# pyannote/pyannote-audio

Measured on AMD Instinct MI355X. Metric: audio-hours/sec (real-time factor) for speaker-diarization-3.1 pipeline, higher is better.
Workload: dtype f32

## Files before the change

### include/pyannote_amd.h

```cpp
#ifndef PYANNOTE_AMD_H
#define PYANNOTE_AMD_H

#include <stddef.h>
#include <stdint.h>

#ifdef __cplusplus
extern "C" {
#endif

int pa_version(void);
const char* pa_last_error(void);

void pa_prof_enable(int on);
size_t pa_prof_report(char* buf, size_t cap);

#define PA_MAX_LSTM_LAYERS 8
#define PA_MAX_LINEAR 4

typedef struct pa_seg_weights {
  int32_t sinc_stride;
  int32_t lstm_layers;
  int32_t lstm_hidden;
  int32_t lstm_bidir;
  int32_t num_linear;
// ... 66 lines not shown
  int32_t bottleneck;
  const float* fb_window;
  const float* fb_tw256;
  const float* fb_tw512;
  const float* fb_mel_w;
  const int32_t* fb_mel_lo;
  const int32_t* fb_mel_hi;
  const float* stem_w;
  const float* stem_shift;
  const float* blk_w1[PA_MAX_RES_BLOCKS];
  const float* blk_shift1[PA_MAX_RES_BLOCKS];
  const float* blk_w2[PA_MAX_RES_BLOCKS];
  const float* blk_shift2[PA_MAX_RES_BLOCKS];
  const float* blk_u1[PA_MAX_RES_BLOCKS];
  const float* blk_u2[PA_MAX_RES_BLOCKS];
  const float* blk_wsc[PA_MAX_RES_BLOCKS];
  const float* blk_shiftsc[PA_MAX_RES_BLOCKS];
  const float* blk_w3[PA_MAX_RES_BLOCKS];
  const float* blk_shift3[PA_MAX_RES_BLOCKS];
  const float* seg1_w;
  const float* seg1_b;
  const float* blk_v1[PA_MAX_RES_BLOCKS];
  const float* blk_v2[PA_MAX_RES_BLOCKS];
  int32_t fb_center_kernel;
} pa_emb_weights;

int pa_emb_num_fbank_frames(int num_samples);
int pa_emb_num_pool_frames(const pa_emb_weights* w, int num_samples);
size_t pa_emb_workspace_bytes(const pa_emb_weights* w, int num_chunks, int num_samples, int num_masks);
int pa_emb_forward(const pa_emb_weights* w, const float* wav, int64_t wav_len, int64_t chunk_stride,
                   int num_chunks, int num_samples, const float* masks, int num_masks, int mask_frames,
                   const int32_t* nearest_idx, float* emb, void* workspace, size_t workspace_bytes,
                   void* stream);

size_t pa_emb_ragged_workspace_bytes(const pa_emb_weights* w, int num_utterances, int max_samples);
int pa_emb_forward_ragged(const pa_emb_weights* w, const float* wav, int64_t wav_len, const int64_t* offsets,
                          const int32_t* lengths, int num_utterances, int max_samples, const float* masks, float* emb,
                          void* workspace, size_t workspace_bytes, void* stream);

size_t pa_emb_calibrate_workspace_bytes(const pa_emb_weights* w, int num_chunks, int num_samples);
int pa_emb_calibrate_winograd(const pa_emb_weights* w, const float* wav, int64_t wav_len, int64_t chunk_stride,
                              int num_chunks, int num_samples, float* report, float* emb, void* workspace,
                              size_t workspace_bytes, void* stream);
int pa_absmax_diff(const float* got, const float* ref, long n, float* out2, void* stream);

int pa_fbank(const float* wav, long wav_len, long chunk_stride, int B, int N, const float* window,
             const float* tw256, const float* tw512, const float* mel_w, const int* mel_lo,
             const int* mel_hi, int nmel, float* out, int center, void* stream);
int pa_fbank_center_span(const float* fb, int B, int T, int nmel, int kernel, float* out, void* stream);
int pa_resnet_stem(const float* fbank, int B, int T, int F, const float* w9, const float* shift,
                   float* out, void* stream);
int pa_conv3x3(const float* X, int B, int H, int W, int cin, const float* Wg, const float* shift,
               const float* R, float* Y, int cout, int stride, int relu, void* stream);
int pa_winograd_pack_host(const float* conv_weight ,
                          const float* bn_scale , int cout, int cin,
                          float* U_slabs );
int pa_conv3x3_wino(const float* X, int B, int H, int W, int cin, const float* U, const float* shift,
                    const float* R, float* Y, int cout, int relu, void* stream);
int pa_winograd4_pack_host(const float* conv_weight ,
                           const float* bn_scale , int cout, int cin,
                           float* U_slabs );
int pa_conv3x3_wino4(const float* X, int B, int H, int W, int cin, const float* U, const float* shift,
                     const float* R, float* Y, int cout, int relu, void* stream);
int pa_conv3x3_wino4_rows(const float* X, int B, int H, int W, int cin, const float* U, const float* shift,
                          const float* R, float* Y, int cout, int relu, int rows, void* stream);
int pa_conv3x3_wino_rows(const float* X, int B, int H, int W, int cin, const float* U, const float* shift,
                         const float* R, float* Y, int cout, int relu, int y_first, void* stream);
int pa_stats_pool(const float* feat, int B, int Fh, int Tp, int C, const float* masks, int S, int Fm,
                  const int* nearest_idx, float* stats, void* stream);
int pa_fbank_ragged(const float* wav, long wav_len, const int64_t* offsets, const int32_t* lengths, int B,
                    int max_samples, const float* window, const float* tw256, const float* tw512, const float* mel_w,
                    const int* mel_lo, const int* mel_hi, int nmel, float* out, void* stream);
int pa_zero_tail_cols(float* x, int B, int H, int W, int C, const int32_t* lengths, int halvings, void* stream);
int pa_stats_pool_ragged(const float* feat, int B, int Fh, int W, int C, const int32_t* lengths, int halvings,
                         const float* masks, int ld_masks, float* stats, void* stream);

#define PA_W2V_MAX_CONV 8
#define PA_W2V_MAX_LAYERS 24
typedef struct pa_w2v_layer {
  const float* qk_w;
  const float* qk_b;
  const float* v_w;
  const float* out_w;
  const float* out_b;
  const float* ln1_g;
  const float* ln1_b;
  const float* ff1_w;
  const float* ff1_b;
  const float* ff2_w;
  const float* ff2_b;
  const float* ln2_g;
  const float* ln2_b;
  const float* gate_w;
  const float* gate_b;
  const float* gate_const;
} pa_w2v_layer;

typedef struct pa_sser_weights {
  int32_t num_conv;
  int32_t conv_channels[PA_W2V_MAX_CONV];
  int32_t conv_kernel[PA_W2V_MAX_CONV];
  int32_t conv_stride[PA_W2V_MAX_CONV];
  int32_t extractor_layer_norm;
  int32_t embed_dim, num_layers, num_heads, ff_dim, layer_norm_first;
  int32_t pos_kernel, pos_groups;
  int32_t wavlm;
// ... 122 lines not shown
```

### pyannote-audio_amd/csrc/emb_forward.cpp

```cpp
#include <hip/hip_runtime.h>
#include <stdint.h>
#include <stdlib.h>

#include "../../include/pyannote_amd.h"

namespace pa {
void set_error(const char* fmt, ...);
}

namespace {

struct EmbPlan {
  int B, N, T, F, S;
  int Hs[5], Ws[5];
  size_t fbank, act[4], stats, total, act_elems;
  size_t t2_off, gather_off;
};
inline size_t align64(size_t n) { return (n + 63) & ~(size_t)63; }

inline bool prefer_wino4(int H, int W, int cin) {
  auto up = [](int a, int b) { return (long)((a + b - 1) / b) * b; };
  long p4 = up(H, 4) * up(W, 64);
  const long p4_lin = up(H, 4) * up(W, 4);
  if (p4_lin * 120 <= p4 * 100) p4 = p4_lin * 120 / 100;
  long p2 = up(H, 8) * up(W, 32);
  if (up(H, 4) * up(W, 64) < p2) p2 = up(H, 4) * up(W, 64);
  if (up(H, 2) * up(W, 128) < p2) p2 = up(H, 2) * up(W, 128);
  const long gain = cin >= 256 ? 130 : 122;
  return p4 * 100 <= p2 * gain;
}

inline bool split_rows_wanted() {
  static const bool on = getenv("PA_EMB_SPLIT_ROWS") != nullptr && atoi(getenv("PA_EMB_SPLIT_ROWS")) != 0;
  return on;
}

bool make_plan(const pa_emb_weights* w, int B, int N, int S, EmbPlan* p, bool calib = false) {
  if (N < 400) return false;
  p->B = B;
  p->N = N;
  p->S = S < 1 ? 1 : S;
  p->T = 1 + (N - 400) / 160;
  p->F = w->num_mel;
  p->Hs[0] = p->F;
  p->Ws[0] = p->T;
  for (int l = 0; l < w->num_layers; ++l) {
    const int s = l == 0 ? 1 : 2;
    p->Hs[l + 1] = (p->Hs[l] - 1) / s + 1;
    p->Ws[l + 1] = (p->Ws[l] - 1) / s + 1;
  }
  size_t o = 0;
  auto take = [&](size_t n) {
    size_t r = o;
    o += align64(n);
    return r;
  };
  p->fbank = take((size_t)B * p->T * p->F);
  const int ex = w->bottleneck ? 4 : 1;
  p->act_elems = (size_t)B * p->Hs[0] * p->Ws[0] * w->planes[0] * ex;
  for (int i = 0; i < 3; ++i) p->act[i] = take(p->act_elems);
  p->t2_off = p->gather_off = 0;
  if (w->bottleneck) {
    size_t t1 = 0, t2 = 0, g = 0;
    int cin = w->planes[0];
    for (int l = 0; l < w->num_layers; ++l) {
      const size_t planes = w->planes[l];
      const size_t in_px = (size_t)B * p->Hs[l == 0 ? 1 : l] * p->Ws[l == 0 ? 1 : l];
      const size_t out_px = (size_t)B * p->Hs[l + 1] * p->Ws[l + 1];
      t1 = t1 > in_px * planes ? t1 : in_px * planes;
      t2 = t2 > out_px * planes ? t2 : out_px * planes;
      if (l > 0) g = g > out_px * cin ? g : out_px * cin;
      cin = 4 * (int)planes;
    }
    p->t2_off = align64(t1);
    p->gather_off = p->t2_off + align64(t2);
    p->act[3] = take(p->gather_off + align64(g));
  } else if (calib) {
    p->act[3] = take(p->act_elems);
  }
  const int L = w->num_layers;
  p->stats = take((size_t)B * p->S * 2 * w->planes[L - 1] * ex * p->Hs[L]);
  p->total = o;
  return true;
}

}
// ... 108 lines not shown
    for (int l = 0; l < w->num_layers; ++l) {
      const int planes = w->planes[l], cout = 4 * planes;
      for (int i = 0; i < w->num_blocks[l]; ++i, ++blk) {
        if (blk >= PA_MAX_RES_BLOCKS) {
          pa::set_error("pa_emb_forward: more than %d residual blocks", PA_MAX_RES_BLOCKS);
          return 3;
        }
        const int stride = (i == 0 && l > 0) ? 2 : 1;
        const int H = stride == 2 ? p.Hs[l] : p.Hs[l + 1], W = stride == 2 ? p.Ws[l] : p.Ws[l + 1];
        const int Ho = p.Hs[l + 1], Wo = p.Ws[l + 1];
        float* t1 = tmp;
        float* t2 = tmp + p.t2_off;
        RUN(pa_gemm_tn_ex(cur, cin, w->blk_w1[blk], cin, w->blk_shift1[blk], nullptr, t1, planes, B * H * W,
                          planes, cin, 2, 0, stream));
        RUN(zero_tail(t1, stride == 2 ? l : l + 1, planes));
        if (stride == 1 && w->blk_u2[blk] != nullptr)
          RUN(pa_conv3x3_wino(t1, B, H, W, planes, w->blk_u2[blk], w->blk_shift2[blk], nullptr, t2, planes, 1,
                              stream));
        else
          RUN(pa_conv3x3(t1, B, H, W, planes, w->blk_w2[blk], w->blk_shift2[blk], nullptr, t2, planes, stride,
                         1, stream));
        const float* res = cur;
        if (w->blk_wsc[blk] != nullptr) {
          if (stride == 2)
            RUN(pa_gemm_tn_s2(cur, B, H, W, cin, w->blk_wsc[blk], cin, w->blk_shiftsc[blk], sc, cout, cout, stream));
          else
            RUN(pa_gemm_tn_ex(cur, cin, w->blk_wsc[blk], cin, w->blk_shiftsc[blk], nullptr, sc, cout,
                              B * Ho * Wo, cout, cin, 0, 0, stream));
          res = sc;
        } else if (stride != 1 || cin != cout) {
          pa::set_error("pa_emb_forward: block %d needs a shortcut conv but none was given", blk);
          return 3;
        }
        RUN(pa_gemm_tn_ex(t2, planes, w->blk_w3[blk], planes, w->blk_shift3[blk], res, nxt, cout, B * Ho * Wo,
                          cout, planes, 2, 0, stream));
        float* t = cur;
        cur = nxt;
        nxt = t;
        cin = cout;
      }
    }
  } else
  for (int l = 0; l < w->num_layers; ++l) {
    const int cout = w->planes[l];
    for (int i = 0; i < w->num_blocks[l]; ++i, ++blk) {
      if (blk >= PA_MAX_RES_BLOCKS) {
        pa::set_error("pa_emb_forward: more than %d residual blocks", PA_MAX_RES_BLOCKS);
        return 3;
      }
      const int stride = (i == 0 && l > 0) ? 2 : 1;
      const int H = stride == 2 ? p.Hs[l] : p.Hs[l + 1], W = stride == 2 ? p.Ws[l] : p.Ws[l + 1];
      const int Ho = p.Hs[l + 1], Wo = p.Ws[l + 1];
      if (w->blk_wsc[blk] != nullptr) {
        RUN(pa_conv3x3(cur, B, H, W, cin, w->blk_w1[blk], w->blk_shift1[blk], nullptr, f1, cout, stride,
                       1, stream));
        RUN(zero_tail(f1, l + 1, cout));
        const size_t q = (size_t)B * Ho * Wo * cin;
        float* R = f2 + ((q + 63) & ~(size_t)63);
        if (stride == 2)
          RUN(pa_gemm_tn_s2(cur, B, H, W, cin, w->blk_wsc[blk], cin, w->blk_shiftsc[blk], R, cout, cout, stream));
        else
          RUN(pa_gemm_tn(cur, cin, w->blk_wsc[blk], cin, w->blk_shiftsc[blk], R, cout, B * Ho * Wo, cout, cin, 0, 0,
                         stream));
        RUN(conv_s1(f1, Ho, Wo, cout, w->blk_v2[blk], w->blk_u2[blk], w->blk_w2[blk], w->blk_shift2[blk], R, cur, cout,
                    2 * blk + 1));
        RUN(zero_tail(cur, l + 1, cout));
      } else {
        if (stride != 1 || cin != cout) {
          pa::set_error("pa_emb_forward: block %d needs a shortcut conv but none was given", blk);
          return 3;
        }
        RUN(conv_s1(cur, H, W, cin, w->blk_v1[blk], w->blk_u1[blk], w->blk_w1[blk], w->blk_shift1[blk], nullptr, f1,
                    cout, 2 * blk));
        RUN(zero_tail(f1, l + 1, cout));
        RUN(conv_s1(f1, H, W, cout, w->blk_v2[blk], w->blk_u2[blk], w->blk_w2[blk], w->blk_shift2[blk], cur, f2, cout,
                    2 * blk + 1));
        RUN(zero_tail(f2, l + 1, cout));
        float* t = cur;
        cur = f2;
        f2 = t;
      }
      cin = cout;
    }
  }
  const int L = w->num_layers;
  const int S = p.S;
  const int cfin = w->planes[L - 1] * (w->bottleneck ? 4 : 1);
  if (ragged)
    RUN(pa_stats_pool_ragged(cur, B, p.Hs[L], p.Ws[L], cfin, lengths, L - 1, masks, p.Ws[L], ws + p.stats, stream));
  else
    RUN(pa_stats_pool(cur, B, p.Hs[L], p.Ws[L], cfin, masks, S, mask_frames, nearest_idx, ws + p.stats, stream));
  const int D2 = 2 * cfin * p.Hs[L];
  RUN(pa_gemm_tn(ws + p.stats, D2, w->seg1_w, D2, w->seg1_b, emb, w->embed_dim, B * S, w->embed_dim, D2,
                 0, 0, stream));
#undef RUN
  return 0;
}

extern "C" {

int pa_emb_forward(const pa_emb_weights* w, const float* wav, int64_t wav_len, int64_t chunk_stride,
                   int num_chunks, int num_samples, const float* masks, int num_masks, int mask_frames,
                   const int32_t* nearest_idx, float* emb, void* workspace, size_t workspace_bytes,
                   void* stream) {
  return emb_forward_impl(w, wav, wav_len, chunk_stride, num_chunks, num_samples, masks, num_masks, mask_frames,
                          nearest_idx, emb, workspace, workspace_bytes, stream, nullptr);
}

size_t pa_emb_ragged_workspace_bytes(const pa_emb_weights* w, int num_utterances, int max_samples) {
  EmbPlan p;
  if (!make_plan(w, num_utterances, max_samples, 1, &p)) return 0;
  return p.total * sizeof(float);
}

int pa_emb_forward_ragged(const pa_emb_weights* w, const float* wav, int64_t wav_len, const int64_t* offsets,
                          const int32_t* lengths, int num_utterances, int max_samples, const float* masks, float* emb,
// ... 29 lines not shown
```

### pyannote-audio_amd/csrc/emb_resnet.hip

```cpp
#include "common.h"
#ifndef PA_CONV_STORE_AUX
#define PA_CONV_STORE_AUX 0
#endif

namespace pa {

constexpr int STEM_TS = 64;
constexpr int STEM_LD = STEM_TS + 3;

__global__ __launch_bounds__(256) void k_stem(const float* __restrict__ fb, int T, int F,
                                              const float* __restrict__ w9,
                                              const float* __restrict__ shift,
                                              float* __restrict__ out) {
  extern __shared__ float xs[];
  const int b = blockIdx.y, t0 = blockIdx.x * STEM_TS;
  const int tid = threadIdx.x;
  for (int i = tid; i < 2 * STEM_LD; i += 256) xs[(i < STEM_LD ? 0 : (F + 1) * STEM_LD - STEM_LD) + i] = 0.f;
  const int n = (STEM_TS + 2) * F;
  for (int i0 = 0; i0 < n; i0 += 8 * 256) {
    float v[8];
#pragma unroll
    for (int k = 0; k < 8; ++k) {
      const int i = i0 + tid + 256 * k;
      const int tt = i / F, ff = i - tt * F, t = t0 + tt - 1;
// ... 27 lines not shown
  float* o = out + ((long)b * F * T + t0 + pl) * 32 + q4;
  for (int f = 0; f < F; ++f) {
#pragma unroll
    for (int h = 0; h < 2; ++h)
#pragma unroll
      for (int dt = 0; dt < 3; ++dt) x2[h][dt] = xs[(f + 2) * STEM_LD + pl + 32 * h + dt];
    float* of = o + (long)f * T * 32;
#pragma unroll
    for (int h = 0; h < 2; ++h) {
      float acc[4];
#pragma unroll
      for (int c = 0; c < 4; ++c) acc[c] = 0.f;
#pragma unroll
      for (int dt = 0; dt < 3; ++dt)
#pragma unroll
        for (int c = 0; c < 4; ++c) acc[c] = fmaf(x0[h][dt], w[dt][c], acc[c]);
#pragma unroll
      for (int dt = 0; dt < 3; ++dt)
#pragma unroll
        for (int c = 0; c < 4; ++c) acc[c] = fmaf(x1[h][dt], w[3 + dt][c], acc[c]);
#pragma unroll
      for (int dt = 0; dt < 3; ++dt)
#pragma unroll
        for (int c = 0; c < 4; ++c) acc[c] = fmaf(x2[h][dt], w[6 + dt][c], acc[c]);
      float4 o4;
      o4.x = fmaxf(acc[0] + sh[0], 0.f);
      o4.y = fmaxf(acc[1] + sh[1], 0.f);
      o4.z = fmaxf(acc[2] + sh[2], 0.f);
      o4.w = fmaxf(acc[3] + sh[3], 0.f);
      if (h == 0 ? ok0 : ok1) *reinterpret_cast<float4*>(of + 32 * 32 * h) = o4;
    }
#pragma unroll
    for (int h = 0; h < 2; ++h)
#pragma unroll
      for (int dt = 0; dt < 3; ++dt) {
        x0[h][dt] = x1[h][dt];
        x1[h][dt] = x2[h][dt];
      }
  }
}

constexpr int CB = 16;
constexpr int CLD = CB + 4;

template <int S, int TH, int TWT>
struct ConvGeom {
  static constexpr int TW = 32 * TWT;
  static constexpr int PH = (TH - 1) * S + 3;
  static constexpr int PW = (TW - 1) * S + 3;
  static constexpr int PWH = ((TW + 1 + 3) / 8) * 8 + 4;
  static constexpr int PATCH = S == 1 ? PH * PW * CLD : PH * 2 * PWH * CLD;
};

template <int S, int TH, int TWT, int BN, bool HAS_R>
__global__ __launch_bounds__(256, 2) void k_conv3x3(const float* __restrict__ X, int H, int W, int CIN,
                                                    const float* __restrict__ Wg,
                                                    const float* __restrict__ shift,
                                                    const float* __restrict__ R, float* __restrict__ Y,
                                                    int Ho, int Wo, int COUT, int relu, int tiles_w,
                                                    int tiles_hw, int n_tiles, int total_tiles, int xranges,
                                                    int* __restrict__ counters) {
  using G = ConvGeom<S, TH, TWT>;
  constexpr int MT = TH * TWT;
  constexpr int MPW = MT / 4;
  constexpr int NT = BN / 32;
  static_assert(MT % 4 == 0, "M-tiles must split over 4 waves");
  extern __shared__ __attribute__((aligned(16))) float smem[];
  float* patch = smem;
  float* wts = smem + G::PATCH;

  const int tid = threadIdx.x, lane = tid & 63, wv = tid >> 6;
  const int li = lane & 31, kh = lane >> 5;
  constexpr int NPF4 = G::PH * G::PW * (CB / 4);
  constexpr int NP = (NPF4 + 255) / 256;
  constexpr int NWF4 = 9 * BN * (CB / 4);
  constexpr int NW = (NWF4 + 255) / 256;
  constexpr int OOB = (int)0x80000000;

  struct Tile {
    int b, n0, y0, x0;
  };
  const int num_pb = total_tiles / n_tiles;
  auto pair_of = [&](int t) {
    return xranges ? (t & 7) * ((num_pb + 7) >> 3) + (t >> 3) / n_tiles : ((t >> 3) / n_tiles) * 8 + (t & 7);
  };
  auto decode = [&](int t) {
    Tile q;
    const int pb = pair_of(t);
    q.n0 = (((t >> 3) % n_tiles)) * BN;
    const int pix = pb % tiles_hw;
    q.b = pb / tiles_hw;
    q.y0 = (pix / tiles_w) * TH;
    q.x0 = (pix % tiles_w) * G::TW;
    return q;
  };
  auto resolve = [&](const TileQueue& tqq, int r) {
    for (;;) {
      const int t = tq_resolve(tqq, r);
      if (t < 0 || pair_of(t) < num_pb) return t;
      r = tq_claim_own(tqq);
    }
  };
  u32x4 rp[NP], rw[NW];
  constexpr bool HOIST = S == 2;
  struct Offs {
    int p[NP];
  };
  int offw[NW];
#pragma unroll
  for (int e = 0; e < NW; ++e) {
    const int i = tid + 256 * e;
    const int c4 = i & 3, rn = i >> 2;
    const int tap = rn / BN, n = rn % BN;
    offw[e] = (NWF4 % 256 == 0 || i < NWF4) ? ((tap * COUT + n) * CIN + 4 * c4) * 4 : OOB;
  }
  auto tile_offsets = [&](const Tile& q, Offs& o) {
#pragma unroll
    for (int e = 0; e < NP; ++e) {
      const int i = tid + 256 * e;
      const int c4 = i & 3, pp = i >> 2;
      const int py = pp / G::PW, px = pp % G::PW;
      const int iy = q.y0 * S - 1 + py, ix = q.x0 * S - 1 + px;
      o.p[e] = ((NPF4 % 256 == 0 || i < NPF4) && iy >= 0 && iy < H && ix >= 0 && ix < W)
                   ? ((iy * W + ix) * CIN + 4 * c4) * 4
                   : OOB;
    }
  };
  auto gload = [&](const Tile& q, const Offs& o, int c0) {
    const __amdgpu_buffer_rsrc_t xsrd = __builtin_amdgcn_make_buffer_rsrc(
        const_cast<float*>(X + (long)q.b * H * W * CIN), 0, H * W * CIN * 4, 0x00020000);
    const __amdgpu_buffer_rsrc_t wsrd = __builtin_amdgcn_make_buffer_rsrc(
        const_cast<float*>(Wg + (long)q.n0 * CIN), 0, (9 * COUT - q.n0) * CIN * 4, 0x00020000);
    Offs here;
    if (!HOIST) tile_offsets(q, here);
#pragma unroll
    for (int e = 0; e < NP; ++e)
      rp[e] = __builtin_amdgcn_raw_buffer_load_b128(xsrd, HOIST ? o.p[e] : here.p[e], c0 * 4, 0);
#pragma unroll
    for (int e = 0; e < NW; ++e) rw[e] = __builtin_amdgcn_raw_buffer_load_b128(wsrd, offw[e], c0 * 4, 0);
  };
  auto lstore = [&]() {
#pragma unroll
    for (int e = 0; e < NP; ++e) {
      const int i = tid + 256 * e;
      const int c4 = i & 3, pp = i >> 2;
      const int py = pp / G::PW, px = pp % G::PW;
      int off;
      if (S == 1) off = pp * CLD + 4 * c4;
      else off = ((py * 2 + (px & 1)) * G::PWH + (px >> 1)) * CLD + 4 * c4;
      if (NPF4 % 256 == 0 || i < NPF4) *reinterpret_cast<u32x4*>(patch + off) = rp[e];
    }
#pragma unroll
    for (int e = 0; e < NW; ++e) {
      const int i = tid + 256 * e;
      if (NWF4 % 256 == 0 || i < NWF4)
        *reinterpret_cast<u32x4*>(wts + (i >> 2) * CLD + 4 * (i & 3)) = rw[e];
    }
  };

  __shared__ int s_next;
  const TileQueue tq{counters, (int)(blockIdx.x & 7), ((num_pb + 7) >> 3) * n_tiles};
  if (tid == 0) s_next = resolve(tq, tq_claim_own(tq));
  __syncthreads();
  int t = s_next;
  if (t < 0) {
    if (tid == 0) tq_done(tq, gridDim.x);
    return;
  }
  Tile cur = decode(t);
  Offs oc, on;
  if (HOIST) tile_offsets(cur, oc);
  on = oc;
  gload(cur, oc, 0);
  for (;;) {
    int ahead = 0;
    if (tid == 0) ahead = tq_claim_own(tq);
    int tn = -1;
    f32x16 acc[MPW][NT];
#pragma unroll
    for (int i = 0; i < MPW; ++i)
#pragma unroll
      for (int j = 0; j < NT; ++j)
#pragma unroll
        for (int r = 0; r < 16; ++r) acc[i][j][r] = 0.f;
    Tile nxt = cur;

    for (int c0 = 0; c0 < CIN; c0 += CB) {
      __syncthreads();
      lstore();
      if (c0 == 0 && tid == 0) s_next = resolve(tq, ahead);
      __syncthreads();
      if (c0 == 0) {
        tn = s_next;
        if (tn >= 0) {
          nxt = decode(tn);
          if (HOIST) tile_offsets(nxt, on);
        }
      }
      if (c0 + CB < CIN) gload(cur, oc, c0 + CB);
      else if (tn >= 0) gload(nxt, on, 0);
      float4 af[1][MPW][2], bf[1][NT][2];
      auto load_tap = [&](int tap, float4 (&a)[MPW][2], float4 (&bq)[NT][2]) {
        const int dy = tap / 3, dx = tap % 3;
#pragma unroll
        for (int i = 0; i < MPW; ++i) {
          const int mt = wv * MPW + i;
          const int yy = mt / TWT, xt = mt % TWT;
          int off;
          if (S == 1) off = ((yy + dy) * G::PW + 32 * xt + li + dx) * CLD;
          else off = (((yy * 2 + dy) * 2 + (dx & 1)) * G::PWH + 32 * xt + li + (dx >> 1)) * CLD;
          a[i][0] = *reinterpret_cast<const float4*>(patch + off + kh * 8);
          a[i][1] = *reinterpret_cast<const float4*>(patch + off + kh * 8 + 4);
        }
#pragma unroll
        for (int j = 0; j < NT; ++j) {
          const int off = (tap * BN + 32 * j + li) * CLD + kh * 8;
          bq[j][0] = *reinterpret_cast<const float4*>(wts + off);
          bq[j][1] = *reinterpret_cast<const float4*>(wts + off + 4);
        }
      };
      auto mfma_tap = [&](const float4 (&a)[MPW][2], const float4 (&bq)[NT][2]) {
#pragma unroll
        for (int h = 0; h < 2; ++h)
#pragma unroll
          for (int i = 0; i < MPW; ++i)
#pragma unroll
            for (int j = 0; j < NT; ++j) {
              acc[i][j] = MFMA32(a[i][h].x, bq[j][h].x, acc[i][j]);
              acc[i][j] = MFMA32(a[i][h].y, bq[j][h].y, acc[i][j]);
              acc[i][j] = MFMA32(a[i][h].z, bq[j][h].z, acc[i][j]);
              acc[i][j] = MFMA32(a[i][h].w, bq[j][h].w, acc[i][j]);
            }
      };
#pragma unroll 1
      for (int dy = 0; dy < 3; ++dy)
#pragma unroll
        for (int dx = 0; dx < 3; ++dx) {
          load_tap(dy * 3 + dx, af[0], bf[0]);
          mfma_tap(af[0], bf[0]);
        }
    }
    {
      const __amdgpu_buffer_rsrc_t ysrd = __builtin_amdgcn_make_buffer_rsrc(
          Y + (long)cur.b * Ho * Wo * COUT, 0, Ho * Wo * COUT * 4, 0x00020000);
      const __amdgpu_buffer_rsrc_t rsrd = __builtin_amdgcn_make_buffer_rsrc(
          const_cast<float*>(HAS_R ? R + (long)cur.b * Ho * Wo * COUT : Y), 0,
          Ho * Wo * COUT * 4, 0x00020000);
      constexpr int NG = MPW * NT;
      int off[2][16];
      float rv[2][16];
      auto goffs = [&](int g, int* o) {
        const int i = g / NT, j = g % NT;
        const int mt = wv * MPW + i;
        const int y = cur.y0 + mt / TWT, xbase = cur.x0 + 32 * (mt % TWT) + 4 * kh;
        const int n = cur.n0 + 32 * j + li;
#pragma unroll
        for (int r = 0; r < 16; ++r) {
          const int x = xbase + (r & 3) + 8 * (r >> 2);
          o[r] = (y < Ho && x < Wo) ? ((y * Wo + x) * COUT + n) * 4 : OOB;
        }
      };
      auto gres = [&](const int* o, float* v) {
        if (HAS_R) {
#pragma unroll
          for (int r = 0; r < 16; ++r)
            v[r] = __builtin_bit_cast(float, __builtin_amdgcn_raw_buffer_load_b32(rsrd, o[r], 0, 0));
        } else {
#pragma unroll
          for (int r = 0; r < 16; ++r) v[r] = 0.f;
        }
      };
      goffs(0, off[0]);
      gres(off[0], rv[0]);
#pragma unroll
      for (int g = 0; g < NG; ++g) {
        if (g + 1 < NG) {
          goffs(g + 1, off[(g + 1) & 1]);
          gres(off[(g + 1) & 1], rv[(g + 1) & 1]);
        }
        const int i = g / NT, j = g % NT;
        const float sh = shift[cur.n0 + 32 * j + li];
#pragma unroll
        for (int r = 0; r < 16; ++r) {
          float v = acc[i][j][r] + sh + rv[g & 1][r];
          if (relu) v = fmaxf(v, 0.f);
          __builtin_amdgcn_raw_buffer_store_b32(__builtin_bit_cast(unsigned int, v), ysrd,
                                                off[g & 1][r], 0, PA_CONV_STORE_AUX);
        }
      }
    }
    if (tn < 0) break;
    cur = nxt;
    oc = on;
  }
  if (tid == 0) tq_done(tq, gridDim.x);
}

int xcd_ranges_wanted(bool by_default);

template <int S, int TH, int TWT, int BN, bool HAS_R>
static int launch_conv_r(const float* X, int B, int H, int W, int CIN, const float* Wg,
                         const float* shift, const float* R, float* Y, int COUT, int relu,
                         hipStream_t st) {
  using G = ConvGeom<S, TH, TWT>;
  const int Ho = (H - 1) / S + 1, Wo = (W - 1) / S + 1;
  const int tiles_w = cdiv(Wo, G::TW), tiles_h = cdiv(Ho, TH);
  const size_t lds = (size_t)(G::PATCH + 9 * BN * CLD) * sizeof(float);
  constexpr int MAXDEV = 16;
  static int resident_of[MAXDEV] = {0}, per_cu_of[MAXDEV] = {0};
  int dev = 0;
  (void)hipGetDevice(&dev);
  if (dev < 0 || dev >= MAXDEV) dev = 0;
  if (!resident_of[dev]) {
    (void)hipFuncSetAttribute((const void*)k_conv3x3<S, TH, TWT, BN, HAS_R>,
                              hipFuncAttributeMaxDynamicSharedMemorySize, (int)lds);
    int cus = 256, per_cu = 2;
    (void)hipDeviceGetAttribute(&cus, hipDeviceAttributeMultiprocessorCount, dev);
    if (hipOccupancyMaxActiveBlocksPerMultiprocessor(&per_cu, k_conv3x3<S, TH, TWT, BN, HAS_R>, 256, lds) !=
            hipSuccess || per_cu < 1)
      per_cu = 2;
    resident_of[dev] = cus * per_cu;
    per_cu_of[dev] = per_cu;
  }
  const int resident = resident_of[dev] & ~7;
  const int tiles_hw = tiles_w * tiles_h, n_tiles = COUT / BN;
  const long total = (long)tiles_hw * n_tiles * B;
  const int grid = (int)(total < resident ? total : resident);
  int* counters = tile_counters();
  if (counters == nullptr) {
    set_error("pa_conv3x3: cannot allocate the tile counters");
    return 2;
  }
  hipLaunchKernelGGL((k_conv3x3<S, TH, TWT, BN, HAS_R>), dim3(grid), dim3(256), lds, st, X, H, W, CIN, Wg,
                     shift, R, Y, Ho, Wo, COUT, relu, tiles_w, tiles_hw, n_tiles, (int)total, xcd_ranges_wanted(true),
                     counters);
  return 0;
}

template <int S, int TH, int TWT, int BN>
static int launch_conv(const float* X, int B, int H, int W, int CIN, const float* Wg,
                       const float* shift, const float* R, float* Y, int COUT, int relu,
                       hipStream_t st) {
  return R != nullptr ? launch_conv_r<S, TH, TWT, BN, true>(X, B, H, W, CIN, Wg, shift, R, Y, COUT, relu, st)
                      : launch_conv_r<S, TH, TWT, BN, false>(X, B, H, W, CIN, Wg, shift, R, Y, COUT, relu, st);
}

}

extern "C" {

int pa_resnet_stem(const float* fbank, int B, int T, int F, const float* w9, const float* shift,
                   float* out, void* stream) {
  if (B <= 0) return 0;
  pa::ProfScope prof("k_stem", stream, 2.0 * B * T * F * 9 * 32, 4.0 * B * T * F * 33);
  PA_REQUIRE(F >= 1 && (size_t)(F + 2) * pa::STEM_LD * 4 <= 64 * 1024, "pa_resnet_stem: %d mel bins do not fit LDS", F);
  hipLaunchKernelGGL(pa::k_stem, dim3(pa::cdiv(T, pa::STEM_TS), B), dim3(256), (size_t)(F + 2) * pa::STEM_LD * 4,
                     (hipStream_t)stream, fbank, T, F, w9, shift, out);
  PA_CHECK_LAUNCH("pa_resnet_stem");
  return 0;
}

int pa_conv3x3(const float* X, int B, int H, int W, int cin, const float* Wg, const float* shift,
               const float* R, float* Y, int cout, int stride, int relu, void* stream) {
  if (B <= 0) return 0;
  PA_REQUIRE(cin % pa::CB == 0 && cout % 32 == 0, "pa_conv3x3: cin %% 16 and cout %% 32 required");
  hipStream_t st = (hipStream_t)stream;
  const int Ho = (H - 1) / stride + 1, Wo_ = (W - 1) / stride + 1;
  pa::ProfScope prof("k_conv3x3", stream, 2.0 * 9 * cin * cout * (double)B * Ho * Wo_,
                     4.0 * ((double)B * H * W * cin + (double)B * Ho * Wo_ * cout * (R ? 2 : 1) + 9.0 * cin * cout));
  if (stride == 1) {
    if (cout == 32) pa::launch_conv<1, 8, 1, 32>(X, B, H, W, cin, Wg, shift, R, Y, cout, relu, st);
    else if (Ho >= 32) pa::launch_conv<1, 8, 1, 64>(X, B, H, W, cin, Wg, shift, R, Y, cout, relu, st);
    else if (Ho >= 16) pa::launch_conv<1, 4, 2, 64>(X, B, H, W, cin, Wg, shift, R, Y, cout, relu, st);
    else pa::launch_conv<1, 2, 2, 64>(X, B, H, W, cin, Wg, shift, R, Y, cout, relu, st);
  } else if (stride == 2) {
    PA_REQUIRE(cout % 64 == 0, "pa_conv3x3: stride 2 needs cout %% 64 == 0");
    if (Ho >= 16) pa::launch_conv<2, 4, 1, 32>(X, B, H, W, cin, Wg, shift, R, Y, cout, relu, st);
    else pa::launch_conv<2, 2, 2, 32>(X, B, H, W, cin, Wg, shift, R, Y, cout, relu, st);
  } else {
    PA_REQUIRE(false, "pa_conv3x3: stride %d not supported", stride);
  }
  PA_CHECK_LAUNCH("pa_conv3x3");
  return 0;
}

}
```

### pyannote-audio_amd/ffi.py

```python
from __future__ import annotations

import ctypes as C
from pathlib import Path

import torch

_LIB = None
PA_MAX_LSTM_LAYERS = 8
PA_MAX_LINEAR = 4

c_fp = C.c_void_p


class SegWeights(C.Structure):
    _fields_ = [
        ("sinc_stride", C.c_int32), ("lstm_layers", C.c_int32), ("lstm_hidden", C.c_int32),
        ("lstm_bidir", C.c_int32), ("num_linear", C.c_int32), ("linear_hidden", C.c_int32),
        ("num_classes", C.c_int32), ("num_speakers", C.c_int32),
        ("wav_gamma", C.c_float), ("wav_beta", C.c_float),
        ("sinc_filt", c_fp), ("norm0", c_fp), ("conv1_w", c_fp), ("conv1_b", c_fp), ("norm1", c_fp),
        ("conv2_w", c_fp), ("conv2_b", c_fp), ("norm2", c_fp),
        ("lstm_wih", c_fp * PA_MAX_LSTM_LAYERS), ("lstm_bias", c_fp * PA_MAX_LSTM_LAYERS),
        ("lstm_whh", c_fp * PA_MAX_LSTM_LAYERS),
        ("lin_w", c_fp * PA_MAX_LINEAR), ("lin_b", c_fp * PA_MAX_LINEAR),
# ... 101 lines not shown
                                   c_fp, c_fp, c_fp, C.c_size_t, c_fp]
    lib.pa_row_stats.argtypes = [c_fp, C.c_long, C.c_long, C.c_int, C.c_int, C.c_float, c_fp, c_fp, c_fp]
    lib.pa_sinc_fir_pool.argtypes = [c_fp, C.c_long, C.c_long, C.c_int, C.c_int, C.c_int, c_fp, c_fp,
                                     C.c_float, C.c_float, c_fp, c_fp, c_fp]
    lib.pa_sinc_fir_span.argtypes = [c_fp, C.c_long, C.c_long, c_fp, c_fp, c_fp]
    lib.pa_sinc_fix_pool.argtypes = [c_fp, C.c_long, C.c_int, C.c_int, C.c_int, c_fp, c_fp, C.c_float, C.c_float,
                                     c_fp, c_fp, c_fp, c_fp]
    lib.pa_conv5_pool.argtypes = [c_fp, C.c_int, C.c_int, C.c_int, c_fp, c_fp, c_fp, c_fp, c_fp, c_fp,
                                  c_fp, c_fp]
    lib.pa_norm_transpose.argtypes = [c_fp, C.c_int, C.c_int, c_fp, c_fp, c_fp, c_fp, c_fp, c_fp]
    lib.pa_gemm_tn_ex.argtypes = [c_fp, C.c_int, c_fp, C.c_int, c_fp, c_fp, c_fp, C.c_long, C.c_int, C.c_int,
                                  C.c_int, C.c_int, C.c_int, c_fp]
    lib.pa_gemm_tn.argtypes = [c_fp, C.c_int, c_fp, C.c_int, c_fp, c_fp, C.c_long, C.c_int, C.c_int,
                               C.c_int, C.c_int, C.c_int, c_fp]
    lib.pa_lstm_rec.argtypes = [c_fp, c_fp, c_fp, C.c_int, C.c_int, C.c_int, c_fp]
    lib.pa_classifier.argtypes = [c_fp, C.c_int, C.c_int, C.c_int, C.c_int, C.c_int, c_fp, c_fp,
                                  C.c_int, c_fp, C.c_int, c_fp, c_fp, c_fp]
    lib.pa_prof_enable.argtypes = [C.c_int]
    lib.pa_prof_enable.restype = None
    lib.pa_prof_report.argtypes = [C.c_char_p, C.c_size_t]
    lib.pa_prof_report.restype = C.c_size_t
    _declare_optional(lib)
    _LIB = lib
    return lib


_OPTIONAL: list[tuple] = [
    ("pa_emb_num_fbank_frames", [C.c_int], C.c_int),
    ("pa_emb_num_pool_frames", [C.POINTER(EmbWeights), C.c_int], C.c_int),
    ("pa_emb_workspace_bytes", [C.POINTER(EmbWeights), C.c_int, C.c_int, C.c_int], C.c_size_t),
    ("pa_emb_forward", [C.POINTER(EmbWeights), c_fp, C.c_int64, C.c_int64, C.c_int, C.c_int, c_fp,
                        C.c_int, C.c_int, c_fp, c_fp, c_fp, C.c_size_t, c_fp], C.c_int),
    ("pa_emb_ragged_workspace_bytes", [C.POINTER(EmbWeights), C.c_int, C.c_int], C.c_size_t),
    ("pa_emb_forward_ragged", [C.POINTER(EmbWeights), c_fp, C.c_int64, c_fp, c_fp, C.c_int, C.c_int, c_fp, c_fp,
                               c_fp, C.c_size_t, c_fp], C.c_int),
    ("pa_fbank_ragged", [c_fp, C.c_long, c_fp, c_fp, C.c_int, C.c_int, c_fp, c_fp, c_fp, c_fp, c_fp, c_fp, C.c_int,
                         c_fp, c_fp], C.c_int),
    ("pa_zero_tail_cols", [c_fp, C.c_int, C.c_int, C.c_int, C.c_int, c_fp, C.c_int, c_fp], C.c_int),
    ("pa_stats_pool_ragged", [c_fp, C.c_int, C.c_int, C.c_int, C.c_int, c_fp, C.c_int, c_fp, C.c_int, c_fp, c_fp],
     C.c_int),
    ("pa_emb_calibrate_workspace_bytes", [C.POINTER(EmbWeights), C.c_int, C.c_int], C.c_size_t),
    ("pa_emb_calibrate_winograd", [C.POINTER(EmbWeights), c_fp, C.c_int64, C.c_int64, C.c_int, C.c_int, c_fp, c_fp,
                                   c_fp, C.c_size_t, c_fp], C.c_int),
    ("pa_lstm_rec_h", [c_fp, c_fp, c_fp, C.c_int, C.c_int, C.c_int, C.c_int, c_fp], C.c_int),
    ("pa_absmax_diff", [c_fp, c_fp, C.c_long, c_fp, c_fp], C.c_int),
    ("pa_gemm_tn_s2", [c_fp, C.c_int, C.c_int, C.c_int, C.c_int, c_fp, C.c_int, c_fp, c_fp, C.c_long, C.c_int,
                       c_fp], C.c_int),
    ("pa_fbank", [c_fp, C.c_long, C.c_long, C.c_int, C.c_int, c_fp, c_fp, c_fp, c_fp, c_fp, c_fp,
                  C.c_int, c_fp, C.c_int, c_fp], C.c_int),
    ("pa_fbank_center_span", [c_fp, C.c_int, C.c_int, C.c_int, C.c_int, c_fp, c_fp], C.c_int),
    ("pa_resnet_stem", [c_fp, C.c_int, C.c_int, C.c_int, c_fp, c_fp, c_fp, c_fp], C.c_int),
    ("pa_conv3x3", [c_fp, C.c_int, C.c_int, C.c_int, C.c_int, c_fp, c_fp, c_fp, c_fp, C.c_int, C.c_int,
                    C.c_int, c_fp], C.c_int),
    ("pa_conv3x3_wino", [c_fp, C.c_int, C.c_int, C.c_int, C.c_int, c_fp, c_fp, c_fp, c_fp, C.c_int, C.c_int,
                         c_fp], C.c_int),
    ("pa_conv3x3_wino4", [c_fp, C.c_int, C.c_int, C.c_int, C.c_int, c_fp, c_fp, c_fp, c_fp, C.c_int, C.c_int,
                          c_fp], C.c_int),
    ("pa_conv3x3_wino4_rows", [c_fp, C.c_int, C.c_int, C.c_int, C.c_int, c_fp, c_fp, c_fp, c_fp, C.c_int, C.c_int,
                               C.c_int, c_fp], C.c_int),
    ("pa_conv3x3_wino_rows", [c_fp, C.c_int, C.c_int, C.c_int, C.c_int, c_fp, c_fp, c_fp, c_fp, C.c_int, C.c_int,
                              C.c_int, c_fp], C.c_int),
    ("pa_pdist_f64", [c_fp, C.c_int, C.c_int, c_fp, c_fp], C.c_int),
    ("pa_cdist_cosine_f64", [c_fp, C.c_int, c_fp, C.c_int, C.c_int, c_fp, c_fp, c_fp], C.c_int),
    ("pa_centroid_means", [c_fp, C.c_int, c_fp, c_fp, C.c_int, c_fp, c_fp], C.c_int),
    ("pa_linkage_workspace_bytes", [C.c_int], C.c_size_t),
    ("pa_linkage_centroid_f64", [c_fp, C.c_int, c_fp, c_fp, C.c_size_t, c_fp], C.c_int),
    ("pa_linkage_centroid_f64_ex", [c_fp, C.c_int, c_fp, c_fp, C.c_size_t, C.c_int, c_fp], C.c_int),
    ("pa_seg_chunk_stats", [c_fp, C.c_int, C.c_int, C.c_int, c_fp, c_fp, c_fp], C.c_int),
    ("pa_embedding_masks", [c_fp, C.c_int, C.c_int, C.c_int, c_fp, C.c_int, C.c_int, c_fp, c_fp], C.c_int),
    ("pa_speaker_count", [c_fp, C.c_int, C.c_int, C.c_int, c_fp, C.c_int, c_fp, c_fp, c_fp], C.c_int),
    ("pa_cluster_activations", [c_fp, C.c_int, C.c_int, C.c_int, c_fp, c_fp, C.c_int, C.c_int, c_fp, c_fp],
     C.c_int),
    ("pa_topk_binarize", [c_fp, c_fp, C.c_int, C.c_int, C.c_int, c_fp, c_fp, c_fp], C.c_int),
    ("pa_topk_binarize_f32", [c_fp, c_fp, C.c_int, C.c_int, C.c_int, c_fp, c_fp, c_fp], C.c_int),
    ("pa_binarize_hysteresis", [c_fp, C.c_int, C.c_int, C.c_int, C.c_float, C.c_float, C.c_int, c_fp, c_fp],
     C.c_int),
    ("pa_cluster_max", [c_fp, C.c_int, C.c_int, C.c_int, c_fp, C.c_int, c_fp, c_fp], C.c_int),
    ("pa_aggregate", [c_fp, C.c_int, C.c_int, C.c_int, c_fp, C.c_int, c_fp, c_fp, C.c_float, C.c_float, C.c_int,
                      c_fp, c_fp], C.c_int),
    ("pa_resample_poly", [c_fp, C.c_long, c_fp, C.c_int, C.c_int, C.c_int, C.c_int, c_fp, C.c_long, c_fp],
     C.c_int),
    ("pa_plda_transform", [c_fp, C.c_int, C.c_int, C.c_int, C.c_int, c_fp, c_fp, c_fp, c_fp, c_fp, c_fp, c_fp],
     C.c_int),
    ("pa_vbx_workspace_bytes", [C.c_int, C.c_int, C.c_int], C.c_size_t),
    ("pa_vbx_iteration", [c_fp, c_fp, C.c_int, C.c_int, C.c_int, C.c_double, C.c_double, C.c_int, c_fp, c_fp,
                          c_fp, C.c_size_t, c_fp], C.c_int),
    ("pa_stats_pool", [c_fp, C.c_int, C.c_int, C.c_int, C.c_int, c_fp, C.c_int, C.c_int, c_fp, c_fp,
                       c_fp], C.c_int),
    ("pa_stats_pool_rows", [c_fp, C.c_int, C.c_int, C.c_int, C.c_int, C.c_int, c_fp, C.c_int, C.c_int, c_fp,
                            c_fp, C.c_int, c_fp, c_fp, c_fp], C.c_int),
    ("pa_sser_num_frames", [C.POINTER(SserWeights), C.c_int], C.c_int),
    ("pa_sser_workspace_bytes", [C.POINTER(SserWeights), C.c_int, C.c_int], C.c_size_t),
    ("pa_sser_forward", [C.POINTER(SserWeights), c_fp, C.c_int64, C.c_int64, C.c_int, C.c_int, c_fp, c_fp, c_fp,
                         c_fp, C.c_size_t, c_fp], C.c_int),
    ("pa_xvec_num_frames", [C.POINTER(XvecWeights), C.c_int], C.c_int),
    ("pa_xvec_workspace_bytes", [C.POINTER(XvecWeights), C.c_int, C.c_int, C.c_int], C.c_size_t),
    ("pa_xvec_forward", [C.POINTER(XvecWeights), c_fp, C.c_int64, C.c_int64, C.c_int, C.c_int, c_fp,
                         C.c_int, C.c_int, c_fp, c_fp, c_fp, C.c_size_t, c_fp], C.c_int),
]


def _declare_optional(lib):
    for name, argtypes, restype in _OPTIONAL:
        if hasattr(lib, name):
            fn = getattr(lib, name)
            fn.argtypes = argtypes
# ... 62 lines not shown
```

Baseline: 1.310.

## Fuse stride-2 shortcut 1x1 conv into entry 3x3 conv kernel

At the entry of each downsampling residual block, the 1x1 stride-2 shortcut projection is now computed inside the 3x3 stride-2 convolution kernel. It reuses the centre-tap input fragments already in registers, with a second accumulator set and an extra LDS slab for the shortcut weights. This removes the separate pa_gemm_tn_s2 launch and its second read of the input activation. In exchange the kernel carries more accumulator registers and LDS, which may reduce occupancy. An environment flag keeps the old path available.

```diff
diff --git a/include/pyannote_amd.h b/include/pyannote_amd.h
--- a/include/pyannote_amd.h
+++ b/include/pyannote_amd.h
@@ -142,6 +142,8 @@
                    float* out, void* stream);
 int pa_conv3x3(const float* X, int B, int H, int W, int cin, const float* Wg, const float* shift,
                const float* R, float* Y, int cout, int stride, int relu, void* stream);
+int pa_conv3x3_s2_entry(const float* X, int B, int H, int W, int cin, const float* Wg, const float* shift,
+                        const float* Wsc, const float* shift_sc, float* Y, float* R, int cout, void* stream);
 int pa_winograd_pack_host(const float* conv_weight ,
                           const float* bn_scale , int cout, int cin,
                           float* U_slabs );
diff --git a/pyannote-audio_amd/csrc/emb_forward.cpp b/pyannote-audio_amd/csrc/emb_forward.cpp
--- a/pyannote-audio_amd/csrc/emb_forward.cpp
+++ b/pyannote-audio_amd/csrc/emb_forward.cpp
@@ -32,6 +32,11 @@
 
 inline bool split_rows_wanted() {
   static const bool on = getenv("PA_EMB_SPLIT_ROWS") != nullptr && atoi(getenv("PA_EMB_SPLIT_ROWS")) != 0;
+  return on;
+}
+
+inline bool fused_entry_wanted() {
+  static const bool on = getenv("PA_EMB_FUSED_ENTRY") == nullptr || atoi(getenv("PA_EMB_FUSED_ENTRY")) != 0;
   return on;
 }
 
@@ -246,16 +251,22 @@
       const int H = stride == 2 ? p.Hs[l] : p.Hs[l + 1], W = stride == 2 ? p.Ws[l] : p.Ws[l + 1];
       const int Ho = p.Hs[l + 1], Wo = p.Ws[l + 1];
       if (w->blk_wsc[blk] != nullptr) {
-        RUN(pa_conv3x3(cur, B, H, W, cin, w->blk_w1[blk], w->blk_shift1[blk], nullptr, f1, cout, stride,
-                       1, stream));
-        RUN(zero_tail(f1, l + 1, cout));
         const size_t q = (size_t)B * Ho * Wo * cin;
         float* R = f2 + ((q + 63) & ~(size_t)63);
-        if (stride == 2)
-          RUN(pa_gemm_tn_s2(cur, B, H, W, cin, w->blk_wsc[blk], cin, w->blk_shiftsc[blk], R, cout, cout, stream));
-        else
-          RUN(pa_gemm_tn(cur, cin, w->blk_wsc[blk], cin, w->blk_shiftsc[blk], R, cout, B * Ho * Wo, cout, cin, 0, 0,
-                         stream));
+        if (stride == 2 && fused_entry_wanted()) {
+          RUN(pa_conv3x3_s2_entry(cur, B, H, W, cin, w->blk_w1[blk], w->blk_shift1[blk], w->blk_wsc[blk],
+                                  w->blk_shiftsc[blk], f1, R, cout, stream));
+          RUN(zero_tail(f1, l + 1, cout));
+        } else {
+          RUN(pa_conv3x3(cur, B, H, W, cin, w->blk_w1[blk], w->blk_shift1[blk], nullptr, f1, cout, stride,
+                         1, stream));
+          RUN(zero_tail(f1, l + 1, cout));
+          if (stride == 2)
+            RUN(pa_gemm_tn_s2(cur, B, H, W, cin, w->blk_wsc[blk], cin, w->blk_shiftsc[blk], R, cout, cout, stream));
+          else
+            RUN(pa_gemm_tn(cur, cin, w->blk_wsc[blk], cin, w->blk_shiftsc[blk], R, cout, B * Ho * Wo, cout, cin, 0,
+                           0, stream));
+        }
         RUN(conv_s1(f1, Ho, Wo, cout, w->blk_v2[blk], w->blk_u2[blk], w->blk_w2[blk], w->blk_shift2[blk], R, cur, cout,
                     2 * blk + 1));
         RUN(zero_tail(cur, l + 1, cout));
diff --git a/pyannote-audio_amd/csrc/emb_resnet.hip b/pyannote-audio_amd/csrc/emb_resnet.hip
--- a/pyannote-audio_amd/csrc/emb_resnet.hip
+++ b/pyannote-audio_amd/csrc/emb_resnet.hip
@@ -103,22 +103,25 @@
   static constexpr int PATCH = S == 1 ? PH * PW * CLD : PH * 2 * PWH * CLD;
 };
 
-template <int S, int TH, int TWT, int BN, bool HAS_R>
+template <int S, int TH, int TWT, int BN, bool HAS_R, bool SC>
 __global__ __launch_bounds__(256, 2) void k_conv3x3(const float* __restrict__ X, int H, int W, int CIN,
                                                     const float* __restrict__ Wg,
                                                     const float* __restrict__ shift,
                                                     const float* __restrict__ R, float* __restrict__ Y,
                                                     int Ho, int Wo, int COUT, int relu, int tiles_w,
                                                     int tiles_hw, int n_tiles, int total_tiles, int xranges,
-                                                    int* __restrict__ counters) {
+                                                    int* __restrict__ counters, const float* __restrict__ Ws,
+                                                    const float* __restrict__ shift_s, float* __restrict__ Rs) {
   using G = ConvGeom<S, TH, TWT>;
   constexpr int MT = TH * TWT;
   constexpr int MPW = MT / 4;
   constexpr int NT = BN / 32;
   static_assert(MT % 4 == 0, "M-tiles must split over 4 waves");
+  static_assert(!SC || (S == 2 && !HAS_R), "the shortcut rides on a stride-2 convolution without residual");
   extern __shared__ __attribute__((aligned(16))) float smem[];
   float* patch = smem;
   float* wts = smem + G::PATCH;
+  float* wsc = wts + 9 * BN * CLD;
 
   const int tid = threadIdx.x, lane = tid & 63, wv = tid >> 6;
   const int li = lane & 31, kh = lane >> 5;
@@ -126,6 +129,8 @@
   constexpr int NP = (NPF4 + 255) / 256;
   constexpr int NWF4 = 9 * BN * (CB / 4);
   constexpr int NW = (NWF4 + 255) / 256;
+  constexpr int NSF4 = BN * (CB / 4);
+  constexpr int NS = SC ? (NSF4 + 255) / 256 : 0;
   constexpr int OOB = (int)0x80000000;
 
   struct Tile {
@@ -152,7 +157,7 @@
       r = tq_claim_own(tqq);
     }
   };
-  u32x4 rp[NP], rw[NW];
+  u32x4 rp[NP], rw[NW], rs[NS > 0 ? NS : 1];
   constexpr bool HOIST = S == 2;
   struct Offs {
     int p[NP];
@@ -164,6 +169,12 @@
     const int c4 = i & 3, rn = i >> 2;
     const int tap = rn / BN, n = rn % BN;
     offw[e] = (NWF4 % 256 == 0 || i < NWF4) ? ((tap * COUT + n) * CIN + 4 * c4) * 4 : OOB;
+  }
+  int offs[NS > 0 ? NS : 1];
+#pragma unroll
+  for (int e = 0; e < NS; ++e) {
+    const int i = tid + 256 * e;
+    offs[e] = (NSF4 % 256 == 0 || i < NSF4) ? ((i >> 2) * CIN + 4 * (i & 3)) * 4 : OOB;
   }
   auto tile_offsets = [&](const Tile& q, Offs& o) {
 #pragma unroll
@@ -189,6 +200,12 @@
       rp[e] = __builtin_amdgcn_raw_buffer_load_b128(xsrd, HOIST ? o.p[e] : here.p[e], c0 * 4, 0);
 #pragma unroll
     for (int e = 0; e < NW; ++e) rw[e] = __builtin_amdgcn_raw_buffer_load_b128(wsrd, offw[e], c0 * 4, 0);
+    if (SC) {
+      const __amdgpu_buffer_rsrc_t ssrd = __builtin_amdgcn_make_buffer_rsrc(
+          const_cast<float*>(Ws + (long)q.n0 * CIN), 0, (COUT - q.n0) * CIN * 4, 0x00020000);
+#pragma unroll
+      for (int e = 0; e < NS; ++e) rs[e] = __builtin_amdgcn_raw_buffer_load_b128(ssrd, offs[e], c0 * 4, 0);
+    }
   };
   auto lstore = [&]() {
 #pragma unroll
@@ -206,6 +223,11 @@
       const int i = tid + 256 * e;
       if (NWF4 % 256 == 0 || i < NWF4)
         *reinterpret_cast<u32x4*>(wts + (i >> 2) * CLD + 4 * (i & 3)) = rw[e];
+    }
+#pragma unroll
+    for (int e = 0; e < NS; ++e) {
+      const int i = tid + 256 * e;
+      if (NSF4 % 256 == 0 || i < NSF4) *reinterpret_cast<u32x4*>(wsc + (i >> 2) * CLD + 4 * (i & 3)) = rs[e];
     }
   };
 
@@ -234,6 +256,15 @@
       for (int j = 0; j < NT; ++j)
 #pragma unroll
         for (int r = 0; r < 16; ++r) acc[i][j][r] = 0.f;
+    f32x16 accs[MPW][NT];
+    if constexpr (SC) {
+#pragma unroll
+      for (int i = 0; i < MPW; ++i)
+#pragma unroll
+        for (int j = 0; j < NT; ++j)
+#pragma unroll
+          for (int r = 0; r < 16; ++r) accs[i][j][r] = 0.f;
+    }
     Tile nxt = cur;
 
     for (int c0 = 0; c0 < CIN; c0 += CB) {
@@ -270,17 +301,17 @@
           bq[j][1] = *reinterpret_cast<const float4*>(wts + off + 4);
         }
       };
-      auto mfma_tap = [&](const float4 (&a)[MPW][2], const float4 (&bq)[NT][2]) {
+      auto mfma_tap = [&](const float4 (&a)[MPW][2], const float4 (&bq)[NT][2], f32x16 (&c)[MPW][NT]) {
 #pragma unroll
         for (int h = 0; h < 2; ++h)
 #pragma unroll
           for (int i = 0; i < MPW; ++i)
 #pragma unroll
             for (int j = 0; j < NT; ++j) {
-              acc[i][j] = MFMA32(a[i][h].x, bq[j][h].x, acc[i][j]);
-              acc[i][j] = MFMA32(a[i][h].y, bq[j][h].y, acc[i][j]);
-              acc[i][j] = MFMA32(a[i][h].z, bq[j][h].z, acc[i][j]);
-              acc[i][j] = MFMA32(a[i][h].w, bq[j][h].w, acc[i][j]);
+              c[i][j] = MFMA32(a[i][h].x, bq[j][h].x, c[i][j]);
+              c[i][j] = MFMA32(a[i][h].y, bq[j][h].y, c[i][j]);
+              c[i][j] = MFMA32(a[i][h].z, bq[j][h].z, c[i][j]);
+              c[i][j] = MFMA32(a[i][h].w, bq[j][h].w, c[i][j]);
             }
       };
 #pragma unroll 1
@@ -288,7 +319,17 @@
 #pragma unroll
         for (int dx = 0; dx < 3; ++dx) {
           load_tap(dy * 3 + dx, af[0], bf[0]);
-          mfma_tap(af[0], bf[0]);
+          mfma_tap(af[0], bf[0], acc);
+          if constexpr (SC) if (dx == 1 && dy == 1) {
+            float4 bs[NT][2];
+#pragma unroll
+            for (int j = 0; j < NT; ++j) {
+              const int off = (32 * j + li) * CLD + kh * 8;
+              bs[j][0] = *reinterpret_cast<const float4*>(wsc + off);
+              bs[j][1] = *reinterpret_cast<const float4*>(wsc + off + 4);
+            }
+            mfma_tap(af[0], bs, accs);
+          }
         }
     }
     {
@@ -297,6 +338,8 @@
       const __amdgpu_buffer_rsrc_t rsrd = __builtin_amdgcn_make_buffer_rsrc(
           const_cast<float*>(HAS_R ? R + (long)cur.b * Ho * Wo * COUT : Y), 0,
           Ho * Wo * COUT * 4, 0x00020000);
+      const __amdgpu_buffer_rsrc_t ssrd = __builtin_amdgcn_make_buffer_rsrc(
+          SC ? Rs + (long)cur.b * Ho * Wo * COUT : Y, 0, Ho * Wo * COUT * 4, 0x00020000);
       constexpr int NG = MPW * NT;
       int off[2][16];
       float rv[2][16];
@@ -338,6 +381,13 @@
           __builtin_amdgcn_raw_buffer_store_b32(__builtin_bit_cast(unsigned int, v), ysrd,
                                                 off[g & 1][r], 0, PA_CONV_STORE_AUX);
         }
+        if constexpr (SC) {
+          const float shs = shift_s[cur.n0 + 32 * j + li];
+#pragma unroll
+          for (int r = 0; r < 16; ++r)
+            __builtin_amdgcn_raw_buffer_store_b32(__builtin_bit_cast(unsigned int, accs[i][j][r] + shs),
+                                                  ssrd, off[g & 1][r], 0, PA_CONV_STORE_AUX);
+        }
       }
     }
     if (tn < 0) break;
@@ -349,25 +399,26 @@
 
 int xcd_ranges_wanted(bool by_default);
 
-template <int S, int TH, int TWT, int BN, bool HAS_R>
+template <int S, int TH, int TWT, int BN, bool HAS_R, bool SC = false>
 static int launch_conv_r(const float* X, int B, int H, int W, int CIN, const float* Wg,
                          const float* shift, const float* R, float* Y, int COUT, int relu,
-                         hipStream_t st) {
+                         hipStream_t st, const float* Ws = nullptr, const float* shift_s = nullptr,
+                         float* Rs = nullptr) {
   using G = ConvGeom<S, TH, TWT>;
   const int Ho = (H - 1) / S + 1, Wo = (W - 1) / S + 1;
   const int tiles_w = cdiv(Wo, G::TW), tiles_h = cdiv(Ho, TH);
-  const size_t lds = (size_t)(G::PATCH + 9 * BN * CLD) * sizeof(float);
+  const size_t lds = (size_t)(G::PATCH + (SC ? 10 : 9) * BN * CLD) * sizeof(float);
   constexpr int MAXDEV = 16;
   static int resident_of[MAXDEV] = {0}, per_cu_of[MAXDEV] = {0};
   int dev = 0;
   (void)hipGetDevice(&dev);
   if (dev < 0 || dev >= MAXDEV) dev = 0;
   if (!resident_of[dev]) {
-    (void)hipFuncSetAttribute((const void*)k_conv3x3<S, TH, TWT, BN, HAS_R>,
+    (void)hipFuncSetAttribute((const void*)k_conv3x3<S, TH, TWT, BN, HAS_R, SC>,
                               hipFuncAttributeMaxDynamicSharedMemorySize, (int)lds);
     int cus = 256, per_cu = 2;
     (void)hipDeviceGetAttribute(&cus, hipDeviceAttributeMultiprocessorCount, dev);
-    if (hipOccupancyMaxActiveBlocksPerMultiprocessor(&per_cu, k_conv3x3<S, TH, TWT, BN, HAS_R>, 256, lds) !=
+    if (hipOccupancyMaxActiveBlocksPerMultiprocessor(&per_cu, k_conv3x3<S, TH, TWT, BN, HAS_R, SC>, 256, lds) !=
             hipSuccess || per_cu < 1)
       per_cu = 2;
     resident_of[dev] = cus * per_cu;
@@ -382,9 +433,9 @@
     set_error("pa_conv3x3: cannot allocate the tile counters");
     return 2;
   }
-  hipLaunchKernelGGL((k_conv3x3<S, TH, TWT, BN, HAS_R>), dim3(grid), dim3(256), lds, st, X, H, W, CIN, Wg,
+  hipLaunchKernelGGL((k_conv3x3<S, TH, TWT, BN, HAS_R, SC>), dim3(grid), dim3(256), lds, st, X, H, W, CIN, Wg,
                      shift, R, Y, Ho, Wo, COUT, relu, tiles_w, tiles_hw, n_tiles, (int)total, xcd_ranges_wanted(true),
-                     counters);
+                     counters, Ws, shift_s, Rs);
   return 0;
 }
 
@@ -435,4 +486,22 @@
   return 0;
 }
 
-}
+int pa_conv3x3_s2_entry(const float* X, int B, int H, int W, int cin, const float* Wg, const float* shift,
+                        const float* Wsc, const float* shift_sc, float* Y, float* R, int cout, void* stream) {
+  if (B <= 0) return 0;
+  PA_REQUIRE(cin % pa::CB == 0 && cout % 64 == 0, "pa_conv3x3_s2_entry: cin %% 16 and cout %% 64 required");
+  PA_REQUIRE(Wsc != nullptr && shift_sc != nullptr && R != nullptr, "pa_conv3x3_s2_entry: the shortcut is required");
+  hipStream_t st = (hipStream_t)stream;
+  const int Ho = (H - 1) / 2 + 1, Wo_ = (W - 1) / 2 + 1;
+  const double P = (double)B * Ho * Wo_;
+  pa::ProfScope prof("k_conv3x3", stream, 2.0 * 10 * cin * cout * P,
+                     4.0 * ((double)B * H * W * cin + 2.0 * P * cout + 10.0 * cin * cout));
+  if (Ho >= 16)
+    pa::launch_conv_r<2, 4, 1, 32, false, true>(X, B, H, W, cin, Wg, shift, nullptr, Y, cout, 1, st, Wsc, shift_sc, R);
+  else
+    pa::launch_conv_r<2, 2, 2, 32, false, true>(X, B, H, W, cin, Wg, shift, nullptr, Y, cout, 1, st, Wsc, shift_sc, R);
+  PA_CHECK_LAUNCH("pa_conv3x3_s2_entry");
+  return 0;
+}
+
+}
diff --git a/pyannote-audio_amd/ffi.py b/pyannote-audio_amd/ffi.py
--- a/pyannote-audio_amd/ffi.py
+++ b/pyannote-audio_amd/ffi.py
@@ -177,6 +177,8 @@
     ("pa_resnet_stem", [c_fp, C.c_int, C.c_int, C.c_int, c_fp, c_fp, c_fp, c_fp], C.c_int),
     ("pa_conv3x3", [c_fp, C.c_int, C.c_int, C.c_int, C.c_int, c_fp, c_fp, c_fp, c_fp, C.c_int, C.c_int,
                     C.c_int, c_fp], C.c_int),
+    ("pa_conv3x3_s2_entry", [c_fp, C.c_int, C.c_int, C.c_int, C.c_int, c_fp, c_fp, c_fp, c_fp, c_fp, c_fp, C.c_int,
+                             c_fp], C.c_int),
     ("pa_conv3x3_wino", [c_fp, C.c_int, C.c_int, C.c_int, C.c_int, c_fp, c_fp, c_fp, c_fp, C.c_int, C.c_int,
                          c_fp], C.c_int),
     ("pa_conv3x3_wino4", [c_fp, C.c_int, C.c_int, C.c_int, C.c_int, c_fp, c_fp, c_fp, c_fp, C.c_int, C.c_int,
```

Result: no change. 1.321, median of 6 (+0.8%).
